# kouyt5/lightning-asr

Measured on AMD Instinct MI355X. Metric: audio-seconds/sec training (asr13x1, bs=32, 10 s clips), higher is better.
Workload: dtype bf16; 1 GPU; asr13x1 QuartzNet-CTC train step, bs=32/GPU, 10 s synthetic 16 kHz clips, labels.txt vocab (C=28), HIP mel+conv+CTC+NovoGrad, random-init weights; global_batch=32, n_class=28, parallelism=dp1, feature_prefetch=True, hip_graph=True, staged_backward=False

## Files before the change

### lightning_asr_amd/csrc/gemm_bf16.hip

```cpp
#include "gemm.h"
#include "reduce_body.h"
#include "lstm_body.h"
#include <algorithm>
#include <stdlib.h>

namespace lasr {

__device__ __forceinline__ void load_bias_quads(const float* __restrict__ bias, int nbase, int N, float (&bv)[2][4][4]) {
#pragma unroll
  for (int ni = 0; ni < 2; ++ni)
#pragma unroll
    for (int j = 0; j < 4; ++j)
#pragma unroll
      for (int e = 0; e < 4; ++e) {
        const int n = nbase + ni * 32 + 8 * j + e;
        bv[ni][j][e] = __uint_as_float(__float_as_uint(bias[min(n, N - 1)]) & (n < N ? 0xffffffffu : 0u));
      }
}


typedef float f32x16 __attribute__((ext_vector_type(16)));
typedef __bf16 bf16x8 __attribute__((ext_vector_type(8)));
typedef short s16x4 __attribute__((ext_vector_type(4)));
typedef short s16x8 __attribute__((ext_vector_type(8)));

static constexpr int TM = 128, TN = 128, TK = 64;
static constexpr int LD_KC = 144;
static constexpr int LD_RC = 320;
static constexpr int OPER_BYTES = 20480;
static constexpr int EPI_LD = 144;

union Frag { uint4 u; s16x8 s; bf16x8 b; };

struct Bf16Args {
  const bf16_t* A; const bf16_t* B; void* C;
  const float* bias; const int32_t* row_lens; float* stat_partials; float* split_ws;
  const bf16_t* addend;
  int M, N, K, lda, ldb, ldc, rows_per_seq, k_per_split;
  int gm, gn, gz;
  int vecA, vecB, vecC;
  const bf16_t* A2; int lda2, K1, act;
  float* row_stat; int32_t* row_arg;
};
struct Bf16Batch { Bf16Args p[2]; int tiles0, total; };

__device__ __forceinline__ uint4 mask_chunk(const uint4& v, int nvalid) {
  const int n = max(0, min(nvalid, 8));
  if (n == 8) return v;
  auto dm = [n](int i) -> uint32_t { return n >= 2 * i + 2 ? 0xffffffffu : (n == 2 * i + 1 ? 0x0000ffffu : 0u); };
  return make_uint4(v.x & dm(0), v.y & dm(1), v.z & dm(2), v.w & dm(3));
}

template <bool TRANS, int ROWS, int NT, int NCH = 4, bool NTL = false>
__device__ __forceinline__ void load_vec(const bf16_t* __restrict__ X, int ld, int R, int r0, int k0, int kend, uint4 (&reg)[NCH]) {
  constexpr int RCH = ROWS / 8;
  const int tid = threadIdx.x;
#pragma unroll
  for (int p = 0; p < NCH; ++p) {
    const int c = tid + NT * p;
    uint32_t off;
    if (!TRANS) off = (uint32_t)min(r0 + (c >> 3), R - 1) * (uint32_t)ld + (uint32_t)min(k0 + ((c & 7) << 3), ((kend + 7) & ~7) - 8);
    else off = (uint32_t)min(k0 + c / RCH, kend - 1) * (uint32_t)ld + (uint32_t)min(r0 + ((c % RCH) << 3), ((R + 7) & ~7) - 8);
    reg[p] = Vec<bf16_t>::raw_if_nt<NTL>(X + off);
  }
}

template <bool TRANS, int ROWS, int NT, int LDK_, int LDR_, int NCH = 4, bool FULL = false>
__device__ __forceinline__ void store_vec(char* __restrict__ s, const uint4 (&reg)[NCH], int k0, int kend) {
  constexpr int RCH = ROWS / 8;
  const int tid = threadIdx.x;
#pragma unroll
  for (int p = 0; p < NCH; ++p) {
    const int c = tid + NT * p;
    const int off = !TRANS ? (c >> 3) * LDK_ + ((c & 7) << 4) : (c / RCH) * LDR_ + ((c % RCH) << 4);
    if constexpr (FULL) {
      *reinterpret_cast<uint4*>(s + off) = reg[p];
    } else {
      const int nvalid = !TRANS ? kend - (k0 + ((c & 7) << 3)) : (k0 + c / RCH < kend ? 8 : 0);
      *reinterpret_cast<uint4*>(s + off) = mask_chunk(reg[p], nvalid);
    }
  }
}

template <bool TRANS, int ROWS, int NT, bool NTL = false>
__device__ __forceinline__ uint4 load_chunk(const bf16_t* __restrict__ X, int ld, int R, int r0, int k0, int kend, int p) {
  constexpr int RCH = ROWS / 8;
  const int c = threadIdx.x + NT * p;
  uint32_t off;
  if (!TRANS) off = (uint32_t)min(r0 + (c >> 3), R - 1) * (uint32_t)ld + (uint32_t)min(k0 + ((c & 7) << 3), ((kend + 7) & ~7) - 8);
  else off = (uint32_t)min(k0 + c / RCH, kend - 1) * (uint32_t)ld + (uint32_t)min(r0 + ((c % RCH) << 3), ((R + 7) & ~7) - 8);
  return Vec<bf16_t>::raw_if_nt<NTL>(X + off);
}
template <bool TRANS, int ROWS, int NT, int LDK_, int LDR_, bool FULL = false>
__device__ __forceinline__ void store_chunk(char* __restrict__ s, const uint4& v, int k0, int kend, int p) {
  constexpr int RCH = ROWS / 8;
  const int c = threadIdx.x + NT * p;
  const int off = !TRANS ? (c >> 3) * LDK_ + ((c & 7) << 4) : (c / RCH) * LDR_ + ((c % RCH) << 4);
  if constexpr (FULL) {
    *reinterpret_cast<uint4*>(s + off) = v;
  } else {
    const int nvalid = !TRANS ? kend - (k0 + ((c & 7) << 3)) : (k0 + c / RCH < kend ? 8 : 0);
    *reinterpret_cast<uint4*>(s + off) = mask_chunk(v, nvalid);
  }
}

template <bool TRANS>
__device__ __forceinline__ void load_oper(const bf16_t* __restrict__ X, int ld, int R, int r0, int k0, int kend, bool vec_ok,
                                          uint4 (&reg)[4]) {
  const int tid = threadIdx.x;
#pragma unroll 1
  for (int p = 0; p < 4; ++p) {
    const int c = tid + 256 * p;
    int row, col, row_lim, col_lim;
    if (!TRANS) { row = r0 + (c >> 3); col = k0 + ((c & 7) << 3); row_lim = R; col_lim = kend; }
    else        { row = k0 + (c >> 4); col = r0 + ((c & 15) << 3); row_lim = kend; col_lim = R; }
    uint4 v = make_uint4(0, 0, 0, 0);
    if (row < row_lim && col < col_lim) {
      const bf16_t* src = X + (uint32_t)row * (uint32_t)ld + (uint32_t)col;
      if (vec_ok && col + 7 < col_lim) {
        v = *reinterpret_cast<const uint4*>(src);
      } else {
        uint32_t w[4] = {0u, 0u, 0u, 0u};
        for (int i = 0; i < 8; ++i)
          if (col + i < col_lim) w[i >> 1] |= (uint32_t)src[i] << (16 * (i & 1));
        v = make_uint4(w[0], w[1], w[2], w[3]);
      }
    }
    if (p == 0) reg[0] = v; else if (p == 1) reg[1] = v; else if (p == 2) reg[2] = v; else reg[3] = v;
  }
}

template <bool TRANS>
__device__ __forceinline__ void store_oper(char* __restrict__ s, const uint4 (&reg)[4]) {
  const int tid = threadIdx.x;
#pragma unroll
  for (int p = 0; p < 4; ++p) {
    const int c = tid + 256 * p;
    const int off = !TRANS ? (c >> 3) * LD_KC + ((c & 7) << 4) : (c >> 4) * LD_RC + ((c & 15) << 4);
    *reinterpret_cast<uint4*>(s + off) = reg[p];
  }
}

template <bool TRANS, int LD_RC_ = LD_RC>
__device__ __forceinline__ bf16x8 load_frag(const char* __restrict__ s, int rb, int ks, int lane) {
  Frag f;
  if (!TRANS) {
    f.u = *reinterpret_cast<const uint4*>(s + (rb + (lane & 31)) * LD_KC + ks * 32 + (lane >> 5) * 16);
  } else {
    const int g = lane >> 4, q = (lane & 15) >> 2, p = lane & 3;
    const int kbase = ks * 16 + 8 * (g >> 1) + q;
    const int col = rb + 16 * (g & 1) + 4 * p;
    typedef __attribute__((address_space(3))) s16x4 lds_s4;
    const char* a0 = s + kbase * LD_RC_ + col * 2;
    const s16x4 lo = __builtin_amdgcn_ds_read_tr16_b64_v4i16((lds_s4*)(a0));
    const s16x4 hi = __builtin_amdgcn_ds_read_tr16_b64_v4i16((lds_s4*)(a0 + 4 * LD_RC_));
    f.s = __builtin_shufflevector(lo, hi, 0, 1, 2, 3, 4, 5, 6, 7);
  }
  return f.b;
}

__device__ __forceinline__ int xcd_remap(int orig, int nwg) {
  const int q = nwg >> 3, r = nwg & 7, xcd = orig & 7;
  return (xcd < r ? xcd * (q + 1) : r * (q + 1) + (xcd - r) * q) + (orig >> 3);
}

typedef float pk_f32x2 __attribute__((ext_vector_type(2)));
typedef __bf16 pk_bf16x2 __attribute__((ext_vector_type(2)));
__device__ __forceinline__ uint32_t pack_bf16x2(float lo, float hi) {
  const pk_f32x2 f = {lo, hi};
  const pk_bf16x2 h = __builtin_convertvector(f, pk_bf16x2);
  return __builtin_bit_cast(uint32_t, h);
}
__device__ __noinline__ void store_bf16_tail(bf16_t* dst, uint4 v, int n) {
  const uint32_t w[4] = {v.x, v.y, v.z, v.w};
#pragma unroll
  for (int i = 0; i < 8; ++i)
    if (i < n) dst[i] = (bf16_t)(w[i >> 1] >> (16 * (i & 1)));
}

template <typename TC, bool TRANS_A, bool TRANS_B, bool VEC>
__device__ __forceinline__ void gemm_bf16_tile(const Bf16Args& g, const int lid) {
  __shared__ __attribute__((aligned(16))) char smem[2 * OPER_BYTES];
  __shared__ float s_stat[2][2][TN];
  __shared__ float s_keep[TM];
  char* sA = smem;
  char* sB = smem + OPER_BYTES;
  const int tid = threadIdx.x, lane = tid & 63, wid = tid >> 6;
  const int wm = wid >> 1, wn = wid & 1;
  const int tn = lid % g.gn, tm = (lid / g.gn) % g.gm, tz = lid / (g.gn * g.gm);
  const int m0 = tm * TM, n0 = tn * TN;
  const int kbeg = tz * g.k_per_split;
  const int kend = min(kbeg + g.k_per_split, g.K);

  if (tid < TM) {
    const int m = m0 + tid;
    bool keep = m < g.M;
    if (keep && g.row_lens) {
      const int b = m / g.rows_per_seq;
      keep = (m - b * g.rows_per_seq) < g.row_lens[b];
    }
    s_keep[tid] = keep ? 1.f : 0.f;
  }

  f32x16 acc[2][2];
#pragma unroll
  for (int i = 0; i < 2; ++i)
#pragma unroll
    for (int j = 0; j < 2; ++j)
#pragma unroll
      for (int r = 0; r < 16; ++r) acc[i][j][r] = 0.f;

  uint4 ra0[4], rb0[4], ra1[4], rb1[4];
#define LASR_LOAD(RA_, RB_, K0_)                                                          \
  if constexpr (VEC) {                                                                   \
    load_vec<TRANS_A, TM, 256>(g.A, g.lda, g.M, m0, (K0_), kend, RA_);                   \
    load_vec<TRANS_B, TN, 256>(g.B, g.ldb, g.N, n0, (K0_), kend, RB_);                   \
  } else {                                                                               \
    load_oper<TRANS_A>(g.A, g.lda, g.M, m0, (K0_), kend, g.vecA, RA_);                   \
    load_oper<TRANS_B>(g.B, g.ldb, g.N, n0, (K0_), kend, g.vecB, RB_);                   \
  }
#define LASR_STORE(RA_, RB_, K0_)                                                         \
  if constexpr (VEC) {                                                                   \
    if ((K0_) + TK <= kend) {              \
      store_vec<TRANS_A, TM, 256, LD_KC, LD_RC, 4, true>(sA, RA_, (K0_), kend);          \
      store_vec<TRANS_B, TN, 256, LD_KC, LD_RC, 4, true>(sB, RB_, (K0_), kend);          \
    } else {                                                                             \
      store_vec<TRANS_A, TM, 256, LD_KC, LD_RC>(sA, RA_, (K0_), kend);                   \
      store_vec<TRANS_B, TN, 256, LD_KC, LD_RC>(sB, RB_, (K0_), kend);                   \
    }                                                                                    \
  } else {                                                                               \
    store_oper<TRANS_A>(sA, RA_);                                                        \
    store_oper<TRANS_B>(sB, RB_);                                                        \
  }
  LASR_LOAD(ra0, rb0, kbeg)
  if (kbeg + TK < kend) { LASR_LOAD(ra1, rb1, kbeg + TK) }
#define LASR_K_STEP(RA_, RB_, KCUR_, KNEXT_)                                              \
  {                                                                                      \
    __syncthreads();                                                                     \
    LASR_STORE(RA_, RB_, KCUR_)                                                          \
    __syncthreads();                                                                     \
    if ((KNEXT_) < kend) { LASR_LOAD(RA_, RB_, KNEXT_) }                                  \
    _Pragma("unroll") for (int ks = 0; ks < TK / 16; ++ks) {                             \
      const bf16x8 a0 = load_frag<TRANS_A>(sA, wm * 64, ks, lane);                       \
      const bf16x8 a1 = load_frag<TRANS_A>(sA, wm * 64 + 32, ks, lane);                  \
      const bf16x8 b0 = load_frag<TRANS_B>(sB, wn * 64, ks, lane);                       \
      const bf16x8 b1 = load_frag<TRANS_B>(sB, wn * 64 + 32, ks, lane);                  \
      acc[0][0] = __builtin_amdgcn_mfma_f32_32x32x16_bf16(b0, a0, acc[0][0], 0, 0, 0);   \
      acc[0][1] = __builtin_amdgcn_mfma_f32_32x32x16_bf16(b1, a0, acc[0][1], 0, 0, 0);   \
      acc[1][0] = __builtin_amdgcn_mfma_f32_32x32x16_bf16(b0, a1, acc[1][0], 0, 0, 0);   \
      acc[1][1] = __builtin_amdgcn_mfma_f32_32x32x16_bf16(b1, a1, acc[1][1], 0, 0, 0);   \
    }                                                                                    \
  }
  for (int k0 = kbeg; k0 < kend; k0 += 2 * TK) {
    LASR_K_STEP(ra0, rb0, k0, k0 + 2 * TK)
    if (k0 + TK < kend) LASR_K_STEP(ra1, rb1, k0 + TK, k0 + 3 * TK)
  }
#undef LASR_LOAD
#undef LASR_STORE
#undef LASR_K_STEP

  const int half = lane >> 5, l31 = lane & 31;
  if constexpr (Elem<TC>::kDtype == LASR_F32) {
    float* W = g.split_ws ? g.split_ws + (size_t)tz * (size_t)g.M * (size_t)g.N : reinterpret_cast<float*>(g.C);
    const int ldw = g.split_ws ? g.N : g.ldc;
    const bool vec4 = (ldw & 3) == 0 && (reinterpret_cast<uintptr_t>(W) & 15) == 0;
    const bool plain = g.split_ws != nullptr;
    const bool has_bias = !plain && g.bias != nullptr;
    float bv[2][4][4];
    if (has_bias) load_bias_quads(g.bias, n0 + wn * 64 + 4 * half, g.N, bv);
#pragma unroll
    for (int mi = 0; mi < 2; ++mi) {
      const int lr = wm * 64 + mi * 32 + l31;
      const int m = m0 + lr;
      const float kf = plain ? 1.f : s_keep[lr];
      if (m < g.M) {
        float* wrow = W + (uint32_t)m * (uint32_t)ldw;
#pragma unroll
        for (int ni = 0; ni < 2; ++ni) {
#pragma unroll
          for (int j = 0; j < 4; ++j) {
            const int n = n0 + wn * 64 + ni * 32 + 8 * j + 4 * half;
            float v[4];
#pragma unroll
            for (int e = 0; e < 4; ++e) {
              v[e] = acc[mi][ni][4 * j + e];
              if (!plain) v[e] = (v[e] + (has_bias ? bv[ni][j][e] : 0.f)) * kf;
            }
            if (vec4 && n + 3 < g.N) {
              *reinterpret_cast<float4*>(wrow + n) = make_float4(v[0], v[1], v[2], v[3]);
            } else {
#pragma unroll
              for (int e = 0; e < 4; ++e)
                if (n + e < g.N) wrow[n + e] = v[e];
            }
          }
        }
      }
    }
  } else {
    uint2 adv[2][2][4];
    const bool has_add = g.addend != nullptr;
    if (has_add) {
#pragma unroll
      for (int mi = 0; mi < 2; ++mi) {
        const uint32_t mrow = (uint32_t)min(m0 + wm * 64 + mi * 32 + l31, g.M - 1) * (uint32_t)g.ldc;
#pragma unroll
        for (int ni = 0; ni < 2; ++ni)
#pragma unroll
          for (int j = 0; j < 4; ++j)
            adv[mi][ni][j] = *reinterpret_cast<const uint2*>(g.addend + mrow + (uint32_t)min(n0 + wn * 64 + ni * 32 + 8 * j + 4 * half, g.N - 4));
      }
    }
    __syncthreads();
    char* epi = smem + wid * (64 * EPI_LD);
    const bool has_bias = g.bias != nullptr;
    float bv[2][4][4];
    if (has_bias) load_bias_quads(g.bias, n0 + wn * 64 + 4 * half, g.N, bv);
#pragma unroll
    for (int mi = 0; mi < 2; ++mi) {
      const uint32_t km = s_keep[wm * 64 + mi * 32 + l31] != 0.f ? 0xffffffffu : 0u;
#pragma unroll
      for (int ni = 0; ni < 2; ++ni) {
#pragma unroll
        for (int j = 0; j < 4; ++j) {
          float v[4];
#pragma unroll
          for (int e = 0; e < 4; ++e) v[e] = acc[mi][ni][4 * j + e];
          if (has_add) {
            const uint2 a = adv[mi][ni][j];
            v[0] += __uint_as_float(a.x << 16); v[1] += __uint_as_float(a.x & 0xffff0000u);
            v[2] += __uint_as_float(a.y << 16); v[3] += __uint_as_float(a.y & 0xffff0000u);
          }
          if (has_bias) {
#pragma unroll
            for (int e = 0; e < 4; ++e) v[e] += bv[ni][j][e];
          }
          uint2 pk;
          pk.x = pack_bf16x2(v[0], v[1]) & km;
          pk.y = pack_bf16x2(v[2], v[3]) & km;
          *reinterpret_cast<uint2*>(epi + (mi * 32 + l31) * EPI_LD + (ni * 32 + 8 * j + 4 * half) * 2) = pk;
        }
      }
    }
    __syncthreads();
    {
      bf16_t* C = reinterpret_cast<bf16_t*>(g.C);
      const int cg = lane & 7, rr = lane >> 3;
      const int n = n0 + wn * 64 + cg * 8;
      const bool full_n = g.vecC && n + 7 < g.N;
      const bool want_stats = g.stat_partials != nullptr;
      float cs[8], cq[8];
#pragma unroll
      for (int i = 0; i < 8; ++i) { cs[i] = 0.f; cq[i] = 0.f; }
#pragma unroll
      for (int it = 0; it < 8; ++it) {
        const int lr = it * 8 + rr;
        const int m = m0 + wm * 64 + lr;
        const uint4 v = *reinterpret_cast<const uint4*>(epi + lr * EPI_LD + cg * 16);
        if (want_stats) {
          const uint32_t w[4] = {v.x, v.y, v.z, v.w};
#pragma unroll
          for (int i = 0; i < 4; ++i) {
            const float x0 = __uint_as_float(w[i] << 16), x1 = __uint_as_float(w[i] & 0xffff0000u);
            cs[2 * i] += x0; cq[2 * i] = fmaf(x0, x0, cq[2 * i]);
            cs[2 * i + 1] += x1; cq[2 * i + 1] = fmaf(x1, x1, cq[2 * i + 1]);
          }
        }
        if (m < g.M && n < g.N) {
          bf16_t* dst = C + (uint32_t)m * (uint32_t)g.ldc + (uint32_t)n;
          if (full_n) *reinterpret_cast<uint4*>(dst) = v;
          else store_bf16_tail(dst, v, min(g.N - n, 8));
        }
      }
      if (want_stats) {
#pragma unroll
        for (int i = 0; i < 8; ++i) {
#pragma unroll
          for (int d = 8; d < 64; d <<= 1) {
            cs[i] += __shfl_xor(cs[i], d, 64);
            cq[i] += __shfl_xor(cq[i], d, 64);
          }
        }
        if (rr == 0) {
#pragma unroll
          for (int i = 0; i < 8; ++i) {
            s_stat[wm][0][wn * 64 + cg * 8 + i] = cs[i];
            s_stat[wm][1][wn * 64 + cg * 8 + i] = cq[i];
          }
        }
      }
    }
    if (g.stat_partials) {
      __syncthreads();
      if (tid < TN) {
        const int n = n0 + tid;
        if (n < g.N) {
          float* P = g.stat_partials + (size_t)tm * 2 * g.N;
          P[n] = s_stat[0][0][tid] + s_stat[1][0][tid];
          P[g.N + n] = s_stat[0][1][tid] + s_stat[1][1][tid];
        }
      }
    }
  }
}

template <typename TC, bool TRANS_A, bool TRANS_B, bool VEC>
__global__ __launch_bounds__(256, 2) void gemm_bf16_kernel(Bf16Batch gb) {
  const int lid_all = xcd_remap(blockIdx.x, gb.total);
  const bool second = lid_all >= gb.tiles0;
  const Bf16Args& g = second ? gb.p[1] : gb.p[0];
  gemm_bf16_tile<TC, TRANS_A, TRANS_B, VEC>(g, second ? lid_all - gb.tiles0 : lid_all);
}

static constexpr int kMaxMulti = 32;
static constexpr int kMaxRiders = 24;
struct Bf16Multi { Bf16Args p[kMaxMulti]; int start[kMaxMulti + 1]; int n, total; lasr_reduce_desc rd[kMaxRiders]; int n_rd, n_rwg; };
template <bool VEC>
__global__ __launch_bounds__(256, 2) void gemm_bf16_multi_kernel(Bf16Multi gm) {
  const int lid_all = xcd_remap(blockIdx.x, gm.total);
  int i = 0;
  while (i + 1 < gm.n && gm.start[i + 1] <= lid_all) ++i;
  gemm_bf16_tile<float, true, true, VEC>(gm.p[i], lid_all - gm.start[i]);
}

namespace big {
static constexpr int BTM = 256, NT = 512;
static constexpr int LDR = 576;
static constexpr int OPER = 36864;
template <bool NARROW>
struct Cfg {
  static constexpr int BN = NARROW ? 128 : 256;
  static constexpr int WN = NARROW ? 2 : 4;
  static constexpr int MI = NARROW ? 2 : 4;
  static constexpr int NCB = BN * 8 / NT;
  static constexpr int LDRB = BN * 2 + 64;
  static constexpr int OPER_B = (BN * LD_KC > 64 * LDRB) ? BN * LD_KC : 64 * LDRB;
  static constexpr int BUF = OPER + OPER_B;
  static constexpr int EPB = BN * 2 + 16;
};
}

__device__ __forceinline__ uint4 load_chunk_dual(const Bf16Args& g, int m0, int k0, int p, const uint32_t (&kma)[4]) {
  const int c = threadIdx.x + big::NT * p;
  const bool first = k0 < g.K1;
  const bf16_t* X = first ? g.A : g.A2;
  const int ld = first ? g.lda : g.lda2;
  const int kk = (first ? k0 : k0 - g.K1) + ((c & 7) << 3);
  (void)kma;
  return *reinterpret_cast<const uint4*>(X + (uint32_t)min(m0 + (c >> 3), g.M - 1) * (uint32_t)ld + (uint32_t)kk);
}
__device__ __forceinline__ uint4 dual_row_mask(const Bf16Args& g, uint4 v, int k0, int p, const uint32_t (&kma)[4]) {
  const uint32_t mk = k0 < g.K1 ? kma[p] : 0xffffffffu;
  return make_uint4(v.x & mk, v.y & mk, v.z & mk, v.w & mk);
}

template <bool TRANS_A, bool TRANS_B, bool NARROW, bool STORE, bool LOAD, bool DUAL = false, bool NTL = false, bool FULLST = false>
__device__ __forceinline__ void big_step(const char* __restrict__ sA, const char* __restrict__ sB, char* __restrict__ dA,
                                         char* __restrict__ dB, f32x16 (&acc)[big::Cfg<NARROW>::MI][2], uint4 (&ra)[4],
                                         uint4 (&rb)[big::Cfg<NARROW>::NCB], const Bf16Args& g, int m0, int n0, int k_store,
                                         int k_load, int kend, int wm, int wn, int lane, const uint32_t (&kma)[4]) {
  using namespace big;
  using CF = Cfg<NARROW>;
  constexpr int MI = CF::MI;
  bf16x8 a[2][MI], b[2][2];
#pragma unroll
  for (int ni = 0; ni < 2; ++ni) b[0][ni] = load_frag<TRANS_B, CF::LDRB>(sB, wn * 64 + ni * 32, 0, lane);
#pragma unroll
  for (int mi = 0; mi < MI; ++mi) a[0][mi] = load_frag<TRANS_A, LDR>(sA, wm * (32 * MI) + mi * 32, 0, lane);
#pragma unroll
  for (int ks = 0; ks < TK / 16; ++ks) {
    const int cur = ks & 1, nxt = cur ^ 1;
    if (ks + 1 < TK / 16) {
#pragma unroll
      for (int ni = 0; ni < 2; ++ni) b[nxt][ni] = load_frag<TRANS_B, CF::LDRB>(sB, wn * 64 + ni * 32, ks + 1, lane);
#pragma unroll
      for (int mi = 0; mi < MI; ++mi) a[nxt][mi] = load_frag<TRANS_A, LDR>(sA, wm * (32 * MI) + mi * 32, ks + 1, lane);
    }
#pragma unroll
    for (int mi = 0; mi < MI; ++mi)
#pragma unroll
      for (int ni = 0; ni < 2; ++ni) acc[mi][ni] = __builtin_amdgcn_mfma_f32_32x32x16_bf16(b[cur][ni], a[cur][mi], acc[mi][ni], 0, 0, 0);
    if constexpr (STORE) {
      if constexpr (DUAL) store_chunk<TRANS_A, BTM, NT, LD_KC, LDR, FULLST>(dA, dual_row_mask(g, ra[ks], k_store, ks, kma), k_store, kend, ks);
      else store_chunk<TRANS_A, BTM, NT, LD_KC, LDR, FULLST>(dA, ra[ks], k_store, kend, ks);
      if constexpr (CF::NCB == 4) store_chunk<TRANS_B, CF::BN, NT, LD_KC, CF::LDRB, FULLST>(dB, rb[ks], k_store, kend, ks);
      else if (ks < CF::NCB) store_chunk<TRANS_B, CF::BN, NT, LD_KC, CF::LDRB, FULLST>(dB, rb[ks < CF::NCB ? ks : 0], k_store, kend, ks);
    }
    if constexpr (LOAD) {
      if constexpr (DUAL) ra[ks] = load_chunk_dual(g, m0, k_load, ks, kma);
      else ra[ks] = load_chunk<TRANS_A, BTM, NT, NTL>(g.A, g.lda, g.M, m0, k_load, kend, ks);
      if constexpr (CF::NCB == 4) rb[ks] = load_chunk<TRANS_B, CF::BN, NT, NTL>(g.B, g.ldb, g.N, n0, k_load, kend, ks);
      else if (ks < CF::NCB) rb[ks < CF::NCB ? ks : 0] = load_chunk<TRANS_B, CF::BN, NT, NTL>(g.B, g.ldb, g.N, n0, k_load, kend, ks);
    }
  }
}

#ifdef LASR_GEMM_STAMPS
__device__ unsigned long long* g_stamps = nullptr;
#define LASR_STAMP(i_) do { if (stamps && threadIdx.x == 0 && blockIdx.x < 4096) stamps[blockIdx.x * 8 + (i_)] = wall_clock64(); } while (0)
#else
#define LASR_STAMP(i_) do {} while (0)
#endif

template <bool TRANS_A, bool TRANS_B, bool NARROW, bool SLAB, bool DUAL = false, bool NTL = false>
__device__ __forceinline__ void gemm_bf16_big_tile(const Bf16Args& g, const int lid) {
#ifdef LASR_GEMM_STAMPS
  unsigned long long* stamps = g_stamps;
#endif
  LASR_STAMP(0);
  using big::BTM; using big::NT; using big::LDR; using big::OPER;
  using CF = big::Cfg<NARROW>;
  constexpr int BTN = CF::BN, BUF = CF::BUF, MI = CF::MI;
  __shared__ __attribute__((aligned(16))) char smem[2 * BUF];
  __shared__ float s_keep[BTM];
  const int tid = threadIdx.x, lane = tid & 63, wid = tid >> 6;
  const int wm = wid / CF::WN, wn = wid % CF::WN;
  const int tn = lid % g.gn, tm = (lid / g.gn) % g.gm, tz = lid / (g.gn * g.gm);
  const int m0 = tm * BTM, n0 = tn * BTN;
  const int kbeg = tz * g.k_per_split;
  const int kend = min(kbeg + g.k_per_split, g.K);
  const int nk = (kend - kbeg + TK - 1) / TK;

  const bool row_masked = !DUAL && g.row_lens != nullptr;
  int keep_pos, keep_len;
  {
    const int m = min(m0 + (tid & (BTM - 1)), g.M - 1);
    const int b = m / g.rows_per_seq;
    keep_pos = m - b * g.rows_per_seq;
    const int32_t* lp = row_masked ? g.row_lens + b : reinterpret_cast<const int32_t*>(g.B);
    keep_len = *lp;
  }

  f32x16 acc[MI][2];
#pragma unroll
  for (int i = 0; i < MI; ++i)
#pragma unroll
    for (int j = 0; j < 2; ++j)
#pragma unroll
      for (int r = 0; r < 16; ++r) acc[i][j][r] = 0.f;

  uint4 ra[4], rb[CF::NCB];
  uint32_t kma[4] = {0xffffffffu, 0xffffffffu, 0xffffffffu, 0xffffffffu};
  if constexpr (DUAL) {
#pragma unroll
    for (int p = 0; p < 4; ++p) {
      const int m = min(m0 + ((tid + NT * p) >> 3), g.M - 1);
      if (g.row_lens) {
        const int b = m / g.rows_per_seq;
        kma[p] = (m - b * g.rows_per_seq) < g.row_lens[b] ? 0xffffffffu : 0u;
      }
    }
#pragma unroll
    for (int p = 0; p < 4; ++p) ra[p] = load_chunk_dual(g, m0, kbeg, p, kma);
  } else {
    load_vec<TRANS_A, BTM, NT, 4, NTL>(g.A, g.lda, g.M, m0, kbeg, kend, ra);
  }
  load_vec<TRANS_B, BTN, NT, CF::NCB, NTL>(g.B, g.ldb, g.N, n0, kbeg, kend, rb);
  if constexpr (DUAL) {
#pragma unroll
    for (int p = 0; p < 4; ++p) ra[p] = dual_row_mask(g, ra[p], kbeg, p, kma);
  }
  store_vec<TRANS_A, BTM, NT, LD_KC, LDR>(smem, ra, kbeg, kend);
  store_vec<TRANS_B, BTN, NT, LD_KC, CF::LDRB, CF::NCB>(smem + OPER, rb, kbeg, kend);
  if (tid < BTM) s_keep[tid] = (m0 + tid < g.M && (!row_masked || keep_pos < keep_len)) ? 1.f : 0.f;
  if (nk > 1) {
    if constexpr (DUAL) {
#pragma unroll
      for (int p = 0; p < 4; ++p) ra[p] = load_chunk_dual(g, m0, kbeg + TK, p, kma);
    } else {
      load_vec<TRANS_A, BTM, NT, 4, NTL>(g.A, g.lda, g.M, m0, kbeg + TK, kend, ra);
    }
    load_vec<TRANS_B, BTN, NT, CF::NCB, NTL>(g.B, g.ldb, g.N, n0, kbeg + TK, kend, rb);
  }
  __syncthreads();
  LASR_STAMP(1);
#ifdef LASR_GEMM_STAMPS
  unsigned long long kstamp_barrier = 0;
  const unsigned long long kstamp_c0 = __builtin_readcyclecounter();
#endif
  {
    int it = 0;
    for (; it + 2 < nk; ++it) {
      const char* sA = smem + (it & 1) * BUF;
      char* dA = smem + ((it + 1) & 1) * BUF;
      big_step<TRANS_A, TRANS_B, NARROW, true, true, DUAL, NTL, true>(sA, sA + OPER, dA, dA + OPER, acc, ra, rb, g, m0, n0, kbeg + (it + 1) * TK,
                                             kbeg + (it + 2) * TK, kend, wm, wn, lane, kma);
#ifdef LASR_GEMM_STAMPS
      asm volatile("s_waitcnt lgkmcnt(0)" ::: "memory");
      const unsigned long long tb0 = __builtin_readcyclecounter();
      __syncthreads();
      kstamp_barrier += __builtin_readcyclecounter() - tb0;
#else
      __syncthreads();
#endif
    }
    if (it + 1 < nk) {
      const char* sA = smem + (it & 1) * BUF;
      char* dA = smem + ((it + 1) & 1) * BUF;
      big_step<TRANS_A, TRANS_B, NARROW, true, false, DUAL>(sA, sA + OPER, dA, dA + OPER, acc, ra, rb, g, m0, n0, kbeg + (it + 1) * TK, 0, kend,
                                              wm, wn, lane, kma);
      __syncthreads();
      ++it;
    }
    const char* sA = smem + (it & 1) * BUF;
    big_step<TRANS_A, TRANS_B, NARROW, false, false, DUAL>(sA, sA + OPER, nullptr, nullptr, acc, ra, rb, g, m0, n0, 0, 0, kend, wm, wn, lane, kma);
    __syncthreads();
  }
  LASR_STAMP(2);
#ifdef LASR_GEMM_STAMPS
  if (stamps && threadIdx.x == 0 && blockIdx.x < 4096) {
    stamps[blockIdx.x * 8 + 6] = __builtin_readcyclecounter() - kstamp_c0;
    stamps[blockIdx.x * 8 + 7] = kstamp_barrier;
  }
#endif
  constexpr int EPB = CF::EPB;
  const int half = lane >> 5, l31 = lane & 31;
  const int nb = n0 + wn * 64;
  if constexpr (SLAB) {
    float* W = g.split_ws + (size_t)tz * (size_t)g.M * (size_t)g.N;
    const bool vec4 = (g.N & 3) == 0;
#pragma unroll
    for (int mi = 0; mi < MI; ++mi) {
      const int m = m0 + wm * (32 * MI) + mi * 32 + l31;
      if (m < g.M) {
        float* wrow = W + (size_t)m * (size_t)g.N;
#pragma unroll
        for (int ni = 0; ni < 2; ++ni) {
#pragma unroll
          for (int j = 0; j < 4; ++j) {
            const int n = nb + ni * 32 + 8 * j + 4 * half;
            if (vec4 && n + 3 < g.N) {
              *reinterpret_cast<float4*>(wrow + n) = make_float4(acc[mi][ni][4 * j], acc[mi][ni][4 * j + 1], acc[mi][ni][4 * j + 2], acc[mi][ni][4 * j + 3]);
            } else {
#pragma unroll
              for (int e = 0; e < 4; ++e)
                if (n + e < g.N) wrow[n + e] = acc[mi][ni][4 * j + e];
            }
          }
        }
      }
    }
    return;
  }
  bf16_t* C = reinterpret_cast<bf16_t*>(g.C);
  {
    char* img = smem + (wm * (32 * MI) + l31) * EPB + (wn * 64 + 4 * half) * 2;
    const bool has_bias = g.bias != nullptr;
    float bv[2][4][4];
    if (has_bias) load_bias_quads(g.bias, nb + 4 * half, g.N, bv);
#pragma unroll
    for (int mi = 0; mi < MI; ++mi) {
      const uint32_t km = s_keep[wm * (32 * MI) + mi * 32 + l31] != 0.f ? 0xffffffffu : 0u;
#pragma unroll
      for (int ni = 0; ni < 2; ++ni) {
#pragma unroll
        for (int j = 0; j < 4; ++j) {
          float v[4];
#pragma unroll
          for (int e = 0; e < 4; ++e) v[e] = acc[mi][ni][4 * j + e];
          if (has_bias) {
#pragma unroll
            for (int e = 0; e < 4; ++e) v[e] += bv[ni][j][e];
          }
          if constexpr (DUAL) {
#pragma unroll
            for (int e = 0; e < 4; ++e) {
              if (g.act == LASR_ACT_RELU) v[e] = fmaxf(v[e], 0.f);
              else if (g.act == LASR_ACT_SWISH) v[e] = v[e] / (1.f + __expf(-v[e]));
            }
          }
          uint2 pk;
          pk.x = pack_bf16x2(v[0], v[1]) & km;
          pk.y = pack_bf16x2(v[2], v[3]) & km;
          *reinterpret_cast<uint2*>(img + mi * 32 * EPB + (ni * 32 + 8 * j) * 2) = pk;
        }
      }
    }
  }
  __syncthreads();
  LASR_STAMP(5);
  constexpr int LPR = BTN / 8, RPI = 64 / LPR, NIT = 32 / RPI;
  const int lc = lane % LPR, lrow = lane / LPR;
  const int nst = n0 + lc * 8;
  const bool full_n = g.vecC && nst + 7 < g.N;
  const bool want_stats = g.stat_partials != nullptr;
  const bool want_rowstat = g.row_stat != nullptr;
  float cs[8], cq[8];
#pragma unroll
  for (int i = 0; i < 8; ++i) { cs[i] = 0.f; cq[i] = 0.f; }
  uint4 vv[NIT];
#pragma unroll
  for (int it = 0; it < NIT; ++it) vv[it] = *reinterpret_cast<const uint4*>(smem + (wid * 32 + it * RPI + lrow) * EPB + lc * 16);
#pragma unroll
  for (int it = 0; it < NIT; ++it) {
    const int lr = wid * 32 + it * RPI + lrow;
    const int m = m0 + lr;
    const uint4 v = vv[it];
    if (want_rowstat) {
      const uint32_t w[4] = {v.x, v.y, v.z, v.w};
      float x[8];
#pragma unroll
      for (int i = 0; i < 4; ++i) { x[2 * i] = __uint_as_float(w[i] << 16); x[2 * i + 1] = __uint_as_float(w[i] & 0xffff0000u); }
      float mx = -INFINITY;
      int mi = 0x7fffffff;
#pragma unroll
      for (int i = 0; i < 8; ++i)
        if (nst + i < g.N && x[i] > mx) { mx = x[i]; mi = nst + i; }
#pragma unroll
      for (int d = 1; d < LPR; d <<= 1) {
        const float om = __shfl_xor(mx, d, 64);
        const int oi = __shfl_xor(mi, d, 64);
        if (om > mx || (om == mx && oi < mi)) { mx = om; mi = oi; }
      }
      float se = 0.f;
#pragma unroll
      for (int i = 0; i < 8; ++i)
        if (nst + i < g.N) se += __expf(x[i] - mx);
#pragma unroll
      for (int d = 1; d < LPR; d <<= 1) se += __shfl_xor(se, d, 64);
      if (lc == 0 && m < g.M) {
        const size_t o = (size_t)m * g.gn + tn;
        g.row_stat[2 * o] = mx; g.row_stat[2 * o + 1] = se; g.row_arg[o] = mi;
      }
    }
    if (want_stats) {
      const uint32_t w[4] = {v.x, v.y, v.z, v.w};
#pragma unroll
      for (int i = 0; i < 4; ++i) {
        const float x0 = __uint_as_float(w[i] << 16), x1 = __uint_as_float(w[i] & 0xffff0000u);
        cs[2 * i] += x0; cq[2 * i] = fmaf(x0, x0, cq[2 * i]);
        cs[2 * i + 1] += x1; cq[2 * i + 1] = fmaf(x1, x1, cq[2 * i + 1]);
      }
    }
    if (m < g.M && nst < g.N) {
      bf16_t* dst = C + (uint32_t)m * (uint32_t)g.ldc + (uint32_t)nst;
      if (full_n) {
        *reinterpret_cast<uint4*>(dst) = v;
      } else {
        store_bf16_tail(dst, v, min(g.N - nst, 8));
      }
    }
  }
  LASR_STAMP(3);
  if (want_stats) {
#pragma unroll
    for (int i = 0; i < 8; ++i) {
#pragma unroll
      for (int d = LPR; d < 64; d <<= 1) {
        cs[i] += __shfl_xor(cs[i], d, 64);
        cq[i] += __shfl_xor(cq[i], d, 64);
      }
    }
    __syncthreads();
    float* s_part = reinterpret_cast<float*>(smem);
    if (lrow == 0) {
#pragma unroll
      for (int i = 0; i < 8; ++i) {
        s_part[(wid * 2 + 0) * BTN + lc * 8 + i] = cs[i];
        s_part[(wid * 2 + 1) * BTN + lc * 8 + i] = cq[i];
      }
    }
    __syncthreads();
    if (tid < BTN) {
      const int n = n0 + tid;
      if (n < g.N) {
        float* P = g.stat_partials + (size_t)tm * 2 * g.N;
        float s0 = 0.f, s1 = 0.f;
#pragma unroll
        for (int w = 0; w < 8; ++w) { s0 += s_part[(w * 2 + 0) * BTN + tid]; s1 += s_part[(w * 2 + 1) * BTN + tid]; }
        P[n] = s0;
        P[g.N + n] = s1;
      }
    }
  }
#ifdef LASR_GEMM_STAMPS
  __builtin_amdgcn_s_waitcnt(0);
  LASR_STAMP(4);
#endif
}

template <bool TRANS_A, bool TRANS_B, bool NARROW>
__global__ __launch_bounds__(512, 1) void gemm_bf16_big_kernel(Bf16Batch gb) {
  const int lid_all = xcd_remap(blockIdx.x, gb.total);
  const bool second = lid_all >= gb.tiles0;
  const Bf16Args& g = second ? gb.p[1] : gb.p[0];
  gemm_bf16_big_tile<TRANS_A, TRANS_B, NARROW, false>(g, second ? lid_all - gb.tiles0 : lid_all);
}

__global__ __launch_bounds__(512, 1) void gemm_bf16_dual_kernel(Bf16Batch gb) {
  gemm_bf16_big_tile<false, false, true, false, true>(gb.p[0], xcd_remap(blockIdx.x, gb.total));
}

template <bool NTL>
__global__ __launch_bounds__(512, 1) void gemm_bf16_big_multi_kernel(Bf16Multi gm) {
  if ((int)blockIdx.x >= gm.total) {
    const int r = blockIdx.x - gm.total;
    for (int s = 0; s < gm.n_rd; ++s) {
      const lasr_reduce_desc q = gm.rd[s];
      for (int64_t i = (int64_t)r * big::NT + threadIdx.x; i < q.n; i += (int64_t)gm.n_rwg * big::NT) reduce_many_elem(q, i);
    }
    return;
  }
  const int lid_all = xcd_remap(blockIdx.x, gm.total);
  int i = 0;
  while (i + 1 < gm.n && gm.start[i + 1] <= lid_all) ++i;
  gemm_bf16_big_tile<true, true, false, true, false, NTL>(gm.p[i], lid_all - gm.start[i]);
}

struct LstmJob { lstm::BwdArgs a; int n_wg; int n_utt; };
template <bool NTL, int KP, bool PAIR>
__global__ __launch_bounds__(512, 1) void gemm_bf16_big_multi_lstm_kernel(Bf16Multi gm, LstmJob job) {
  if ((int)blockIdx.x < job.n_wg) {
    __shared__ lstm::BwdSmem sm[2];
    const int slot = threadIdx.x / 192;
    if (slot >= (PAIR ? 2 : 1)) return;
    const int b = PAIR ? blockIdx.x : blockIdx.x >> 1, dir = PAIR ? slot : (blockIdx.x & 1);
    lstm::bilstm_bwd_body<bf16_t, true, KP>(job.a, b, dir, (int)threadIdx.x - slot * 192, 192, sm[slot], [] { lds_barrier(); });
    return;
  }
  const int lid_all = xcd_remap((int)blockIdx.x - job.n_wg, gm.total);
  int i = 0;
  while (i + 1 < gm.n && gm.start[i + 1] <= lid_all) ++i;
// ... 183 lines not shown
```

Measured before the change: 154,100 audio-seconds/sec.

## Switch bf16 GEMMs to 16x16x32 MFMA with swizzled LDS K-layout

Result: faster. 156,600 audio-seconds/sec (median of 6 runs) (+1.6%).

```diff
diff --git a/lightning_asr_amd/csrc/gemm_bf16.hip b/lightning_asr_amd/csrc/gemm_bf16.hip
--- a/lightning_asr_amd/csrc/gemm_bf16.hip
+++ b/lightning_asr_amd/csrc/gemm_bf16.hip
@@ -6,20 +6,18 @@
 
 namespace lasr {
 
-__device__ __forceinline__ void load_bias_quads(const float* __restrict__ bias, int nbase, int N, float (&bv)[2][4][4]) {
-#pragma unroll
-  for (int ni = 0; ni < 2; ++ni)
-#pragma unroll
-    for (int j = 0; j < 4; ++j)
-#pragma unroll
-      for (int e = 0; e < 4; ++e) {
-        const int n = nbase + ni * 32 + 8 * j + e;
-        bv[ni][j][e] = __uint_as_float(__float_as_uint(bias[min(n, N - 1)]) & (n < N ? 0xffffffffu : 0u));
-      }
-}
-
-
-typedef float f32x16 __attribute__((ext_vector_type(16)));
+__device__ __forceinline__ void load_bias_quads(const float* __restrict__ bias, int nbase, int N, float (&bv)[4][4]) {
+#pragma unroll
+  for (int ni = 0; ni < 4; ++ni)
+#pragma unroll
+    for (int e = 0; e < 4; ++e) {
+      const int n = nbase + ni * 16 + e;
+      bv[ni][e] = __uint_as_float(__float_as_uint(bias[min(n, N - 1)]) & (n < N ? 0xffffffffu : 0u));
+    }
+}
+
+
+typedef float f32x4 __attribute__((ext_vector_type(4)));
 typedef __bf16 bf16x8 __attribute__((ext_vector_type(8)));
 typedef short s16x4 __attribute__((ext_vector_type(4)));
 typedef short s16x8 __attribute__((ext_vector_type(8)));
@@ -44,6 +42,8 @@
 };
 struct Bf16Batch { Bf16Args p[2]; int tiles0, total; };
 
+__device__ __forceinline__ int kc_slot(int row, int ch) { return ch ^ (((row >> 2) ^ (row >> 3)) & 1); }
+
 __device__ __forceinline__ uint4 mask_chunk(const uint4& v, int nvalid) {
   const int n = max(0, min(nvalid, 8));
   if (n == 8) return v;
@@ -72,7 +72,7 @@
 #pragma unroll
   for (int p = 0; p < NCH; ++p) {
     const int c = tid + NT * p;
-    const int off = !TRANS ? (c >> 3) * LDK_ + ((c & 7) << 4) : (c / RCH) * LDR_ + ((c % RCH) << 4);
+    const int off = !TRANS ? (c >> 3) * LDK_ + (kc_slot(c >> 3, c & 7) << 4) : (c / RCH) * LDR_ + ((c % RCH) << 4);
     if constexpr (FULL) {
       *reinterpret_cast<uint4*>(s + off) = reg[p];
     } else {
@@ -95,7 +95,7 @@
 __device__ __forceinline__ void store_chunk(char* __restrict__ s, const uint4& v, int k0, int kend, int p) {
   constexpr int RCH = ROWS / 8;
   const int c = threadIdx.x + NT * p;
-  const int off = !TRANS ? (c >> 3) * LDK_ + ((c & 7) << 4) : (c / RCH) * LDR_ + ((c % RCH) << 4);
+  const int off = !TRANS ? (c >> 3) * LDK_ + (kc_slot(c >> 3, c & 7) << 4) : (c / RCH) * LDR_ + ((c % RCH) << 4);
   if constexpr (FULL) {
     *reinterpret_cast<uint4*>(s + off) = v;
   } else {
@@ -136,7 +136,7 @@
 #pragma unroll
   for (int p = 0; p < 4; ++p) {
     const int c = tid + 256 * p;
-    const int off = !TRANS ? (c >> 3) * LD_KC + ((c & 7) << 4) : (c >> 4) * LD_RC + ((c & 15) << 4);
+    const int off = !TRANS ? (c >> 3) * LD_KC + (kc_slot(c >> 3, c & 7) << 4) : (c >> 4) * LD_RC + ((c & 15) << 4);
     *reinterpret_cast<uint4*>(s + off) = reg[p];
   }
 }
@@ -145,11 +145,11 @@
 __device__ __forceinline__ bf16x8 load_frag(const char* __restrict__ s, int rb, int ks, int lane) {
   Frag f;
   if (!TRANS) {
-    f.u = *reinterpret_cast<const uint4*>(s + (rb + (lane & 31)) * LD_KC + ks * 32 + (lane >> 5) * 16);
+    f.u = *reinterpret_cast<const uint4*>(s + (rb + (lane & 15)) * LD_KC + ks * 64 + kc_slot(lane & 15, lane >> 4) * 16);
   } else {
     const int g = lane >> 4, q = (lane & 15) >> 2, p = lane & 3;
-    const int kbase = ks * 16 + 8 * (g >> 1) + q;
-    const int col = rb + 16 * (g & 1) + 4 * p;
+    const int kbase = ks * 32 + 8 * g + q;
+    const int col = rb + 4 * p;
     typedef __attribute__((address_space(3))) s16x4 lds_s4;
     const char* a0 = s + kbase * LD_RC_ + col * 2;
     const s16x4 lo = __builtin_amdgcn_ds_read_tr16_b64_v4i16((lds_s4*)(a0));
@@ -202,13 +202,13 @@
     s_keep[tid] = keep ? 1.f : 0.f;
   }
 
-  f32x16 acc[2][2];
-#pragma unroll
-  for (int i = 0; i < 2; ++i)
-#pragma unroll
-    for (int j = 0; j < 2; ++j)
-#pragma unroll
-      for (int r = 0; r < 16; ++r) acc[i][j][r] = 0.f;
+  f32x4 acc[4][4];
+#pragma unroll
+  for (int i = 0; i < 4; ++i)
+#pragma unroll
+    for (int j = 0; j < 4; ++j)
+#pragma unroll
+      for (int r = 0; r < 4; ++r) acc[i][j][r] = 0.f;
 
   uint4 ra0[4], rb0[4], ra1[4], rb1[4];
 #define LASR_LOAD(RA_, RB_, K0_)                                                          \
@@ -240,15 +240,15 @@
     LASR_STORE(RA_, RB_, KCUR_)                                                          \
     __syncthreads();                                                                     \
     if ((KNEXT_) < kend) { LASR_LOAD(RA_, RB_, KNEXT_) }                                  \
-    _Pragma("unroll") for (int ks = 0; ks < TK / 16; ++ks) {                             \
-      const bf16x8 a0 = load_frag<TRANS_A>(sA, wm * 64, ks, lane);                       \
-      const bf16x8 a1 = load_frag<TRANS_A>(sA, wm * 64 + 32, ks, lane);                  \
-      const bf16x8 b0 = load_frag<TRANS_B>(sB, wn * 64, ks, lane);                       \
-      const bf16x8 b1 = load_frag<TRANS_B>(sB, wn * 64 + 32, ks, lane);                  \
-      acc[0][0] = __builtin_amdgcn_mfma_f32_32x32x16_bf16(b0, a0, acc[0][0], 0, 0, 0);   \
-      acc[0][1] = __builtin_amdgcn_mfma_f32_32x32x16_bf16(b1, a0, acc[0][1], 0, 0, 0);   \
-      acc[1][0] = __builtin_amdgcn_mfma_f32_32x32x16_bf16(b0, a1, acc[1][0], 0, 0, 0);   \
-      acc[1][1] = __builtin_amdgcn_mfma_f32_32x32x16_bf16(b1, a1, acc[1][1], 0, 0, 0);   \
+    _Pragma("unroll") for (int ks = 0; ks < TK / 32; ++ks) {                             \
+      bf16x8 a[4], b[4];                                                                 \
+      _Pragma("unroll") for (int i = 0; i < 4; ++i) {                                    \
+        a[i] = load_frag<TRANS_A>(sA, wm * 64 + i * 16, ks, lane);                       \
+        b[i] = load_frag<TRANS_B>(sB, wn * 64 + i * 16, ks, lane);                       \
+      }                                                                                  \
+      _Pragma("unroll") for (int mi = 0; mi < 4; ++mi)                                   \
+        _Pragma("unroll") for (int ni = 0; ni < 4; ++ni)                                 \
+          acc[mi][ni] = __builtin_amdgcn_mfma_f32_16x16x32_bf16(b[ni], a[mi], acc[mi][ni], 0, 0, 0); \
     }                                                                                    \
   }
   for (int k0 = kbeg; k0 < kend; k0 += 2 * TK) {
@@ -259,87 +259,79 @@
 #undef LASR_STORE
 #undef LASR_K_STEP
 
-  const int half = lane >> 5, l31 = lane & 31;
+  const int g4 = lane >> 4, l15 = lane & 15;
   if constexpr (Elem<TC>::kDtype == LASR_F32) {
     float* W = g.split_ws ? g.split_ws + (size_t)tz * (size_t)g.M * (size_t)g.N : reinterpret_cast<float*>(g.C);
     const int ldw = g.split_ws ? g.N : g.ldc;
     const bool vec4 = (ldw & 3) == 0 && (reinterpret_cast<uintptr_t>(W) & 15) == 0;
     const bool plain = g.split_ws != nullptr;
     const bool has_bias = !plain && g.bias != nullptr;
-    float bv[2][4][4];
-    if (has_bias) load_bias_quads(g.bias, n0 + wn * 64 + 4 * half, g.N, bv);
-#pragma unroll
-    for (int mi = 0; mi < 2; ++mi) {
-      const int lr = wm * 64 + mi * 32 + l31;
+    float bv[4][4];
+    if (has_bias) load_bias_quads(g.bias, n0 + wn * 64 + 4 * g4, g.N, bv);
+#pragma unroll
+    for (int mi = 0; mi < 4; ++mi) {
+      const int lr = wm * 64 + mi * 16 + l15;
       const int m = m0 + lr;
       const float kf = plain ? 1.f : s_keep[lr];
       if (m < g.M) {
         float* wrow = W + (uint32_t)m * (uint32_t)ldw;
 #pragma unroll
-        for (int ni = 0; ni < 2; ++ni) {
-#pragma unroll
-          for (int j = 0; j < 4; ++j) {
-            const int n = n0 + wn * 64 + ni * 32 + 8 * j + 4 * half;
-            float v[4];
-#pragma unroll
-            for (int e = 0; e < 4; ++e) {
-              v[e] = acc[mi][ni][4 * j + e];
-              if (!plain) v[e] = (v[e] + (has_bias ? bv[ni][j][e] : 0.f)) * kf;
-            }
-            if (vec4 && n + 3 < g.N) {
-              *reinterpret_cast<float4*>(wrow + n) = make_float4(v[0], v[1], v[2], v[3]);
-            } else {
-#pragma unroll
-              for (int e = 0; e < 4; ++e)
-                if (n + e < g.N) wrow[n + e] = v[e];
-            }
+        for (int ni = 0; ni < 4; ++ni) {
+          const int n = n0 + wn * 64 + ni * 16 + 4 * g4;
+          float v[4];
+#pragma unroll
+          for (int e = 0; e < 4; ++e) {
+            v[e] = acc[mi][ni][e];
+            if (!plain) v[e] = (v[e] + (has_bias ? bv[ni][e] : 0.f)) * kf;
+          }
+          if (vec4 && n + 3 < g.N) {
+            *reinterpret_cast<float4*>(wrow + n) = make_float4(v[0], v[1], v[2], v[3]);
+          } else {
+#pragma unroll
+            for (int e = 0; e < 4; ++e)
+              if (n + e < g.N) wrow[n + e] = v[e];
           }
         }
       }
     }
   } else {
-    uint2 adv[2][2][4];
+    uint2 adv[4][4];
     const bool has_add = g.addend != nullptr;
     if (has_add) {
 #pragma unroll
-      for (int mi = 0; mi < 2; ++mi) {
-        const uint32_t mrow = (uint32_t)min(m0 + wm * 64 + mi * 32 + l31, g.M - 1) * (uint32_t)g.ldc;
-#pragma unroll
-        for (int ni = 0; ni < 2; ++ni)
-#pragma unroll
-          for (int j = 0; j < 4; ++j)
-            adv[mi][ni][j] = *reinterpret_cast<const uint2*>(g.addend + mrow + (uint32_t)min(n0 + wn * 64 + ni * 32 + 8 * j + 4 * half, g.N - 4));
+      for (int mi = 0; mi < 4; ++mi) {
+        const uint32_t mrow = (uint32_t)min(m0 + wm * 64 + mi * 16 + l15, g.M - 1) * (uint32_t)g.ldc;
+#pragma unroll
+        for (int ni = 0; ni < 4; ++ni)
+          adv[mi][ni] = *reinterpret_cast<const uint2*>(g.addend + mrow + (uint32_t)min(n0 + wn * 64 + ni * 16 + 4 * g4, g.N - 4));
       }
     }
     __syncthreads();
     char* epi = smem + wid * (64 * EPI_LD);
     const bool has_bias = g.bias != nullptr;
-    float bv[2][4][4];
-    if (has_bias) load_bias_quads(g.bias, n0 + wn * 64 + 4 * half, g.N, bv);
-#pragma unroll
-    for (int mi = 0; mi < 2; ++mi) {
-      const uint32_t km = s_keep[wm * 64 + mi * 32 + l31] != 0.f ? 0xffffffffu : 0u;
-#pragma unroll
-      for (int ni = 0; ni < 2; ++ni) {
-#pragma unroll
-        for (int j = 0; j < 4; ++j) {
-          float v[4];
-#pragma unroll
-          for (int e = 0; e < 4; ++e) v[e] = acc[mi][ni][4 * j + e];
-          if (has_add) {
-            const uint2 a = adv[mi][ni][j];
-            v[0] += __uint_as_float(a.x << 16); v[1] += __uint_as_float(a.x & 0xffff0000u);
-            v[2] += __uint_as_float(a.y << 16); v[3] += __uint_as_float(a.y & 0xffff0000u);
-          }
-          if (has_bias) {
-#pragma unroll
-            for (int e = 0; e < 4; ++e) v[e] += bv[ni][j][e];
-          }
-          uint2 pk;
-          pk.x = pack_bf16x2(v[0], v[1]) & km;
-          pk.y = pack_bf16x2(v[2], v[3]) & km;
-          *reinterpret_cast<uint2*>(epi + (mi * 32 + l31) * EPI_LD + (ni * 32 + 8 * j + 4 * half) * 2) = pk;
+    float bv[4][4];
+    if (has_bias) load_bias_quads(g.bias, n0 + wn * 64 + 4 * g4, g.N, bv);
+#pragma unroll
+    for (int mi = 0; mi < 4; ++mi) {
+      const uint32_t km = s_keep[wm * 64 + mi * 16 + l15] != 0.f ? 0xffffffffu : 0u;
+#pragma unroll
+      for (int ni = 0; ni < 4; ++ni) {
+        float v[4];
+#pragma unroll
+        for (int e = 0; e < 4; ++e) v[e] = acc[mi][ni][e];
+        if (has_add) {
+          const uint2 a = adv[mi][ni];
+          v[0] += __uint_as_float(a.x << 16); v[1] += __uint_as_float(a.x & 0xffff0000u);
+          v[2] += __uint_as_float(a.y << 16); v[3] += __uint_as_float(a.y & 0xffff0000u);
         }
+        if (has_bias) {
+#pragma unroll
+          for (int e = 0; e < 4; ++e) v[e] += bv[ni][e];
+        }
+        uint2 pk;
+        pk.x = pack_bf16x2(v[0], v[1]) & km;
+        pk.y = pack_bf16x2(v[2], v[3]) & km;
+        *reinterpret_cast<uint2*>(epi + (mi * 16 + l15) * EPI_LD + (ni * 16 + 4 * g4) * 2) = pk;
       }
     }
     __syncthreads();
@@ -431,7 +423,7 @@
 struct Cfg {
   static constexpr int BN = NARROW ? 128 : 256;
   static constexpr int WN = NARROW ? 2 : 4;
-  static constexpr int MI = NARROW ? 2 : 4;
+  static constexpr int MI = NARROW ? 4 : 8;
   static constexpr int NCB = BN * 8 / NT;
   static constexpr int LDRB = BN * 2 + 64;
   static constexpr int OPER_B = (BN * LD_KC > 64 * LDRB) ? BN * LD_KC : 64 * LDRB;
@@ -456,41 +448,49 @@
 
 template <bool TRANS_A, bool TRANS_B, bool NARROW, bool STORE, bool LOAD, bool DUAL = false, bool NTL = false, bool FULLST = false>
 __device__ __forceinline__ void big_step(const char* __restrict__ sA, const char* __restrict__ sB, char* __restrict__ dA,
-                                         char* __restrict__ dB, f32x16 (&acc)[big::Cfg<NARROW>::MI][2], uint4 (&ra)[4],
+                                         char* __restrict__ dB, f32x4 (&acc)[big::Cfg<NARROW>::MI][4], uint4 (&ra)[4],
                                          uint4 (&rb)[big::Cfg<NARROW>::NCB], const Bf16Args& g, int m0, int n0, int k_store,
                                          int k_load, int kend, int wm, int wn, int lane, const uint32_t (&kma)[4]) {
   using namespace big;
   using CF = Cfg<NARROW>;
   constexpr int MI = CF::MI;
-  bf16x8 a[2][MI], b[2][2];
-#pragma unroll
-  for (int ni = 0; ni < 2; ++ni) b[0][ni] = load_frag<TRANS_B, CF::LDRB>(sB, wn * 64 + ni * 32, 0, lane);
-#pragma unroll
-  for (int mi = 0; mi < MI; ++mi) a[0][mi] = load_frag<TRANS_A, LDR>(sA, wm * (32 * MI) + mi * 32, 0, lane);
-#pragma unroll
-  for (int ks = 0; ks < TK / 16; ++ks) {
-    const int cur = ks & 1, nxt = cur ^ 1;
-    if (ks + 1 < TK / 16) {
-#pragma unroll
-      for (int ni = 0; ni < 2; ++ni) b[nxt][ni] = load_frag<TRANS_B, CF::LDRB>(sB, wn * 64 + ni * 32, ks + 1, lane);
-#pragma unroll
-      for (int mi = 0; mi < MI; ++mi) a[nxt][mi] = load_frag<TRANS_A, LDR>(sA, wm * (32 * MI) + mi * 32, ks + 1, lane);
-    }
-#pragma unroll
-    for (int mi = 0; mi < MI; ++mi)
-#pragma unroll
-      for (int ni = 0; ni < 2; ++ni) acc[mi][ni] = __builtin_amdgcn_mfma_f32_32x32x16_bf16(b[cur][ni], a[cur][mi], acc[mi][ni], 0, 0, 0);
+  constexpr int NG = MI;
+  constexpr int GPC = NG / 4;
+  bf16x8 a[2][2], b[2][4];
+#pragma unroll
+  for (int ni = 0; ni < 4; ++ni) b[0][ni] = load_frag<TRANS_B, CF::LDRB>(sB, wn * 64 + ni * 16, 0, lane);
+#pragma unroll
+  for (int h = 0; h < 2; ++h) a[0][h] = load_frag<TRANS_A, LDR>(sA, wm * (16 * MI) + h * 16, 0, lane);
+#pragma unroll
+  for (int gi = 0; gi < NG; ++gi) {
+    const int ks = gi / (MI / 2), mp = gi % (MI / 2);
+    if (gi + 1 < NG) {
+      const int ks1 = (gi + 1) / (MI / 2), mp1 = (gi + 1) % (MI / 2);
+      if (mp1 == 0) {
+#pragma unroll
+        for (int ni = 0; ni < 4; ++ni) b[ks1 & 1][ni] = load_frag<TRANS_B, CF::LDRB>(sB, wn * 64 + ni * 16, ks1, lane);
+      }
+#pragma unroll
+      for (int h = 0; h < 2; ++h) a[(gi + 1) & 1][h] = load_frag<TRANS_A, LDR>(sA, wm * (16 * MI) + (2 * mp1 + h) * 16, ks1, lane);
+    }
+#pragma unroll
+    for (int h = 0; h < 2; ++h)
+#pragma unroll
+      for (int ni = 0; ni < 4; ++ni)
+        acc[2 * mp + h][ni] = __builtin_amdgcn_mfma_f32_16x16x32_bf16(b[ks & 1][ni], a[gi & 1][h], acc[2 * mp + h][ni], 0, 0, 0);
+    if (gi % GPC != GPC - 1) continue;
+    const int c = gi / GPC;
     if constexpr (STORE) {
-      if constexpr (DUAL) store_chunk<TRANS_A, BTM, NT, LD_KC, LDR, FULLST>(dA, dual_row_mask(g, ra[ks], k_store, ks, kma), k_store, kend, ks);
-      else store_chunk<TRANS_A, BTM, NT, LD_KC, LDR, FULLST>(dA, ra[ks], k_store, kend, ks);
-      if constexpr (CF::NCB == 4) store_chunk<TRANS_B, CF::BN, NT, LD_KC, CF::LDRB, FULLST>(dB, rb[ks], k_store, kend, ks);
-      else if (ks < CF::NCB) store_chunk<TRANS_B, CF::BN, NT, LD_KC, CF::LDRB, FULLST>(dB, rb[ks < CF::NCB ? ks : 0], k_store, kend, ks);
+      if constexpr (DUAL) store_chunk<TRANS_A, BTM, NT, LD_KC, LDR, FULLST>(dA, dual_row_mask(g, ra[c], k_store, c, kma), k_store, kend, c);
+      else store_chunk<TRANS_A, BTM, NT, LD_KC, LDR, FULLST>(dA, ra[c], k_store, kend, c);
+      if constexpr (CF::NCB == 4) store_chunk<TRANS_B, CF::BN, NT, LD_KC, CF::LDRB, FULLST>(dB, rb[c], k_store, kend, c);
+      else if (c < CF::NCB) store_chunk<TRANS_B, CF::BN, NT, LD_KC, CF::LDRB, FULLST>(dB, rb[c < CF::NCB ? c : 0], k_store, kend, c);
     }
     if constexpr (LOAD) {
-      if constexpr (DUAL) ra[ks] = load_chunk_dual(g, m0, k_load, ks, kma);
-      else ra[ks] = load_chunk<TRANS_A, BTM, NT, NTL>(g.A, g.lda, g.M, m0, k_load, kend, ks);
-      if constexpr (CF::NCB == 4) rb[ks] = load_chunk<TRANS_B, CF::BN, NT, NTL>(g.B, g.ldb, g.N, n0, k_load, kend, ks);
-      else if (ks < CF::NCB) rb[ks < CF::NCB ? ks : 0] = load_chunk<TRANS_B, CF::BN, NT, NTL>(g.B, g.ldb, g.N, n0, k_load, kend, ks);
+      if constexpr (DUAL) ra[c] = load_chunk_dual(g, m0, k_load, c, kma);
+      else ra[c] = load_chunk<TRANS_A, BTM, NT, NTL>(g.A, g.lda, g.M, m0, k_load, kend, c);
+      if constexpr (CF::NCB == 4) rb[c] = load_chunk<TRANS_B, CF::BN, NT, NTL>(g.B, g.ldb, g.N, n0, k_load, kend, c);
+      else if (c < CF::NCB) rb[c < CF::NCB ? c : 0] = load_chunk<TRANS_B, CF::BN, NT, NTL>(g.B, g.ldb, g.N, n0, k_load, kend, c);
     }
   }
 }
@@ -513,7 +513,7 @@
   constexpr int BTN = CF::BN, BUF = CF::BUF, MI = CF::MI;
   __shared__ __attribute__((aligned(16))) char smem[2 * BUF];
   __shared__ float s_keep[BTM];
-  const int tid = threadIdx.x, lane = tid & 63, wid = tid >> 6;
+  const int tid = threadIdx.x, lane = __lane_id(), wid = __builtin_amdgcn_readfirstlane(tid >> 6);
   const int wm = wid / CF::WN, wn = wid % CF::WN;
   const int tn = lid % g.gn, tm = (lid / g.gn) % g.gm, tz = lid / (g.gn * g.gm);
   const int m0 = tm * BTM, n0 = tn * BTN;
@@ -531,13 +531,13 @@
     keep_len = *lp;
   }
 
-  f32x16 acc[MI][2];
+  f32x4 acc[MI][4];
 #pragma unroll
   for (int i = 0; i < MI; ++i)
 #pragma unroll
-    for (int j = 0; j < 2; ++j)
-#pragma unroll
-      for (int r = 0; r < 16; ++r) acc[i][j][r] = 0.f;
+    for (int j = 0; j < 4; ++j)
+#pragma unroll
+      for (int r = 0; r < 4; ++r) acc[i][j][r] = 0.f;
 
   uint4 ra[4], rb[CF::NCB];
   uint32_t kma[4] = {0xffffffffu, 0xffffffffu, 0xffffffffu, 0xffffffffu};
@@ -614,28 +614,25 @@
   }
 #endif
   constexpr int EPB = CF::EPB;
-  const int half = lane >> 5, l31 = lane & 31;
+  const int g4 = lane >> 4, l15 = lane & 15;
   const int nb = n0 + wn * 64;
   if constexpr (SLAB) {
     float* W = g.split_ws + (size_t)tz * (size_t)g.M * (size_t)g.N;
     const bool vec4 = (g.N & 3) == 0;
 #pragma unroll
     for (int mi = 0; mi < MI; ++mi) {
-      const int m = m0 + wm * (32 * MI) + mi * 32 + l31;
+      const int m = m0 + wm * (16 * MI) + mi * 16 + l15;
       if (m < g.M) {
         float* wrow = W + (size_t)m * (size_t)g.N;
 #pragma unroll
-        for (int ni = 0; ni < 2; ++ni) {
-#pragma unroll
-          for (int j = 0; j < 4; ++j) {
-            const int n = nb + ni * 32 + 8 * j + 4 * half;
-            if (vec4 && n + 3 < g.N) {
-              *reinterpret_cast<float4*>(wrow + n) = make_float4(acc[mi][ni][4 * j], acc[mi][ni][4 * j + 1], acc[mi][ni][4 * j + 2], acc[mi][ni][4 * j + 3]);
-            } else {
-#pragma unroll
-              for (int e = 0; e < 4; ++e)
-                if (n + e < g.N) wrow[n + e] = acc[mi][ni][4 * j + e];
-            }
+        for (int ni = 0; ni < 4; ++ni) {
+          const int n = nb + ni * 16 + 4 * g4;
+          if (vec4 && n + 3 < g.N) {
+            *reinterpret_cast<float4*>(wrow + n) = make_float4(acc[mi][ni][0], acc[mi][ni][1], acc[mi][ni][2], acc[mi][ni][3]);
+          } else {
+#pragma unroll
+            for (int e = 0; e < 4; ++e)
+              if (n + e < g.N) wrow[n + e] = acc[mi][ni][e];
           }
         }
       }
@@ -644,36 +641,33 @@
   }
   bf16_t* C = reinterpret_cast<bf16_t*>(g.C);
   {
-    char* img = smem + (wm * (32 * MI) + l31) * EPB + (wn * 64 + 4 * half) * 2;
+    char* img = smem + (wm * (16 * MI) + l15) * EPB + (wn * 64 + 4 * g4) * 2;
     const bool has_bias = g.bias != nullptr;
-    float bv[2][4][4];
-    if (has_bias) load_bias_quads(g.bias, nb + 4 * half, g.N, bv);
+    float bv[4][4];
+    if (has_bias) load_bias_quads(g.bias, nb + 4 * g4, g.N, bv);
 #pragma unroll
     for (int mi = 0; mi < MI; ++mi) {
-      const uint32_t km = s_keep[wm * (32 * MI) + mi * 32 + l31] != 0.f ? 0xffffffffu : 0u;
-#pragma unroll
-      for (int ni = 0; ni < 2; ++ni) {
-#pragma unroll
-        for (int j = 0; j < 4; ++j) {
-          float v[4];
-#pragma unroll
-          for (int e = 0; e < 4; ++e) v[e] = acc[mi][ni][4 * j + e];
-          if (has_bias) {
-#pragma unroll
-            for (int e = 0; e < 4; ++e) v[e] += bv[ni][j][e];
+      const uint32_t km = s_keep[wm * (16 * MI) + mi * 16 + l15] != 0.f ? 0xffffffffu : 0u;
+#pragma unroll
+      for (int ni = 0; ni < 4; ++ni) {
+        float v[4];
+#pragma unroll
+        for (int e = 0; e < 4; ++e) v[e] = acc[mi][ni][e];
+        if (has_bias) {
+#pragma unroll
+          for (int e = 0; e < 4; ++e) v[e] += bv[ni][e];
+        }
+        if constexpr (DUAL) {
+#pragma unroll
+          for (int e = 0; e < 4; ++e) {
+            if (g.act == LASR_ACT_RELU) v[e] = fmaxf(v[e], 0.f);
+            else if (g.act == LASR_ACT_SWISH) v[e] = v[e] / (1.f + __expf(-v[e]));
           }
-          if constexpr (DUAL) {
-#pragma unroll
-            for (int e = 0; e < 4; ++e) {
-              if (g.act == LASR_ACT_RELU) v[e] = fmaxf(v[e], 0.f);
-              else if (g.act == LASR_ACT_SWISH) v[e] = v[e] / (1.f + __expf(-v[e]));
-            }
-          }
-          uint2 pk;
-          pk.x = pack_bf16x2(v[0], v[1]) & km;
-          pk.y = pack_bf16x2(v[2], v[3]) & km;
-          *reinterpret_cast<uint2*>(img + mi * 32 * EPB + (ni * 32 + 8 * j) * 2) = pk;
         }
+        uint2 pk;
+        pk.x = pack_bf16x2(v[0], v[1]) & km;
+        pk.y = pack_bf16x2(v[2], v[3]) & km;
+        *reinterpret_cast<uint2*>(img + mi * 16 * EPB + ni * 16 * 2) = pk;
       }
     }
   }
@@ -761,13 +755,14 @@
       }
     }
     __syncthreads();
-    if (tid < BTN) {
-      const int n = n0 + tid;
+    const int t = wid * 64 + lane;
+    if (t < BTN) {
+      const int n = n0 + t;
       if (n < g.N) {
         float* P = g.stat_partials + (size_t)tm * 2 * g.N;
         float s0 = 0.f, s1 = 0.f;
 #pragma unroll
-        for (int w = 0; w < 8; ++w) { s0 += s_part[(w * 2 + 0) * BTN + tid]; s1 += s_part[(w * 2 + 1) * BTN + tid]; }
+        for (int w = 0; w < 8; ++w) { s0 += s_part[(w * 2 + 0) * BTN + t]; s1 += s_part[(w * 2 + 1) * BTN + t]; }
         P[n] = s0;
         P[g.N + n] = s1;
       }
```
